# hlesmqh/WS3D

Hardware: AMD Instinct MI355X
Metric: KITTI scenes/sec (16384 pts) Stage-1 RPN fwd, 1/2/4/8 GPU; FPS+group HBM GB/s (higher is better)
Workload: dtype f32

## Files before the change

### include/ws3d_ops.h

```cpp
#ifndef WS3D_OPS_H
#define WS3D_OPS_H

#include <stddef.h>
#include <stdint.h>

#ifdef __cplusplus
extern "C" {
#endif

#define WS3D_OK 0
#define WS3D_E_INVALID (-1)
#define WS3D_E_LAUNCH (-2)
#define WS3D_E_WORKSPACE (-3)
#define WS3D_E_UNSUPPORTED (-4)

#if defined(__GNUC__)
#define WS3D_API __attribute__((visibility("default")))
#else
#define WS3D_API
#endif

typedef void *ws3d_stream_t;

#define WS3D_ABI_VERSION 6
// ... 168 lines not shown
                                        size_t workspace_bytes, ws3d_stream_t stream);
WS3D_API int ws3d_three_interpolate_grad_det(int b, int c, int n, int m, const float *grad_out, const int32_t *idx,
                                             const float *weight, float *grad_points, void *workspace,
                                             size_t workspace_bytes, ws3d_stream_t stream);

WS3D_API int ws3d_bias_act_inplace(int b, int o_ch, long l, int relu, float *y, const float *bias,
                                   ws3d_stream_t stream);

WS3D_API int ws3d_rowmax_bias_act(int b, int o_ch, long m, int s, int relu, const float *y, const float *bias,
                                  float *out, ws3d_stream_t stream);

WS3D_API int ws3d_query_and_group_nlc(int b, int n, int m, int c, float radius, int nsample, int use_xyz,
                                      const float *xyz, const float *new_xyz, const float *features_nlc,
                                      int32_t *idx_out, float *out_nlc, const void *sorted, ws3d_stream_t stream);
WS3D_API int ws3d_three_interpolate_nlc(int b, int c, int m, int n, const float *feats_nlc, const int32_t *idx,
                                        const float *weight, float *out_nlc, int out_stride, ws3d_stream_t stream);
WS3D_API int ws3d_rowmax_rows(long rows_out, int ns, int o_ch, const float *y, float *out, int out_stride,
                              ws3d_stream_t stream);

WS3D_API int ws3d_sa_mlp3_pool(long rows, int nsample, int c1, int c2, int c3, const float *x_rows4,
                               const float *w1t, const float *b1, const float *w2t, const float *b2,
                               const float *w3t, const float *b3, int relu3, float *out, int out_stride,
                               ws3d_stream_t stream);

WS3D_API int ws3d_mlp2_rows(long rows, int k_dim, int o1, int o2, const float *x_rows, const float *w1t, const float *b1, int relu1,
                   const float *w2t, const float *b2, int relu2, float *out, int *ticket, ws3d_stream_t stream);

WS3D_API size_t ws3d_rpn_heads_blob_bytes(int o2);
WS3D_API int ws3d_rpn_heads_pack(int o2, const float *w1t, const float *b1, int relu1, const float *w2t, const float *b2, int relu2, void *blob,
                        ws3d_stream_t stream);
WS3D_API int ws3d_rpn_heads(long rows, const float *x_rows, int heads, const void *blob_cls, float *out_cls, int *ticket_cls, int o2_reg,
                   const void *blob_reg, float *out_reg, int *ticket_reg, int workgroups, ws3d_stream_t stream);

WS3D_API int ws3d_qinterp_gemm(int b, int n, int m, int c, int o_dim, const float *q, const int32_t *idx, const float *weight, const float *lin,
                      const float *skip, int c1, const float *wb, const float *b1, int relu1, const float *w2t, const float *b2, int relu2,
                      float *out, ws3d_stream_t stream);


WS3D_API int ws3d_boxes_overlap_bev(int num_a, const float *boxes_a, int num_b, const float *boxes_b,
                           float *ans, ws3d_stream_t stream);

WS3D_API int ws3d_boxes_iou_bev(int num_a, const float *boxes_a, int num_b, const float *boxes_b,
                       float *ans, ws3d_stream_t stream);

WS3D_API int ws3d_nms_mask(int boxes_num, const float *boxes, float thresh, int normal, int full_grid,
                  uint64_t *mask, ws3d_stream_t stream);

WS3D_API size_t ws3d_nms_workspace_bytes(int boxes_num);
WS3D_API int ws3d_nms(int boxes_num, const float *boxes, float thresh, int normal, int max_keep,
                      void *workspace, size_t workspace_bytes, int64_t *keep, int32_t *num_keep,
                      ws3d_stream_t stream);

WS3D_API int ws3d_nms_batched(int batch, int boxes_num, const float *boxes, float thresh, int normal,
                              int max_keep, void *workspace, size_t workspace_bytes, int64_t *keep,
                              int32_t *num_keep, ws3d_stream_t stream);


WS3D_API int ws3d_radius_nms_batched(int batch, int n, const float *centers, float radius, int max_keep,
                                     void *workspace, size_t workspace_bytes, int64_t *keep,
                                     int32_t *num_keep, ws3d_stream_t stream);

WS3D_API int ws3d_topk_sorted(int b, int n, int k, const float *scores, float *out_scores, int64_t *out_idx,
                              ws3d_stream_t stream);
WS3D_API size_t ws3d_topk_workspace_bytes(int b, int n);
WS3D_API int ws3d_topk_sorted_ws(int b, int n, int k, const float *scores, float *out_scores, int64_t *out_idx, void *workspace,
                                 size_t workspace_bytes, ws3d_stream_t stream);
// ... 78 lines not shown
```

### ws3d_amd/_lib.py

```python
from __future__ import annotations

import ctypes as C
import os

_HERE = os.path.dirname(os.path.abspath(__file__))
DIST_MODE = int(os.environ.get("WS3D_DIST_MODE", "0") or 0)
LIB_PATH = os.environ.get("WS3D_HIP_LIB") or os.path.join(
    _HERE, "libws3d_hip.so" if DIST_MODE == 0 else "libws3d_hip_dm%d.so" % DIST_MODE)

E_INVALID, E_LAUNCH, E_WORKSPACE, E_UNSUPPORTED = -1, -2, -3, -4
ABI_VERSION = 6

_vp = C.c_void_p
_i = C.c_int
_f = C.c_float
_sz = C.c_size_t

class CompactMlpArgs(C.Structure):
    _fields_ = [("b", _i), ("n", _i), ("m", _i), ("max_rows", C.c_long), ("o1", _i), ("o2", _i), ("o3", _i), ("pmat", _vp), ("p_stride", _i),
                ("xyz", _vp), ("new_xyz", _vp), ("rowc", _vp), ("rowsrc", _vp), ("total", _vp), ("w1x", _vp), ("b1", _vp), ("relu1", _i),
                ("w2t", _vp), ("b2", _vp), ("relu2", _i), ("w3t", _vp), ("b3", _vp), ("mid", _vp), ("out", _vp), ("out_stride", _i), ("limit", C.c_long)]


SIGNATURES = {
# ... 14 lines not shown
    "ws3d_ball_query_pairs2": (_i, [_i, _i, _i, _vp, _vp, _vp, C.c_float, _i, _vp, _vp, _vp, _vp, C.c_float, _i, _vp, _vp, _vp, _vp, _vp]),
    "ws3d_sorted_points_bytes": (_sz, [_i, _i]),
    "ws3d_sort_points_x": (_i, [_i, _i, _vp, _vp, _vp]),
    "ws3d_sort_points_xz": (_i, [_i, _i, _vp, _vp, _vp]),
    "ws3d_sort_points_grid": (_i, [_i, _i, _vp, _vp, _vp]),
    "ws3d_sort_points_jobs": (_i, [_i, _i, _vp, _vp, _vp, _vp, _vp]),
    "ws3d_group_points": (_i, [_i, _i, _i, _i, _i, _vp, _vp, _vp, _vp]),
    "ws3d_group_points_grad": (_i, [_i, _i, _i, _i, _i, _vp, _vp, _vp, _vp]),
    "ws3d_query_and_group": (_i, [_i, _i, _i, _i, _f, _i, _i, _vp, _vp, _vp, _vp, _vp, _vp, _vp]),
    "ws3d_three_nn": (_i, [_i, _i, _i, _vp, _vp, _vp, _vp, _vp, _vp]),
    "ws3d_three_interpolate": (_i, [_i, _i, _i, _i, _vp, _vp, _vp, _vp, _vp]),
    "ws3d_three_interpolate_grad": (_i, [_i, _i, _i, _i, _vp, _vp, _vp, _vp, _vp]),
    "ws3d_bn_workspace_bytes": (C.c_size_t, [_i, _i, C.c_long]),
    "ws3d_bn_relu_train_fwd": (_i, [_i, _i, C.c_long, _vp, _vp, _vp, C.c_float, C.c_float, _i, _vp, _vp, _vp, _vp, _vp, _vp,
                                    _vp, C.c_size_t, _vp]),
    "ws3d_bn_relu_train_bwd": (_i, [_i, _i, C.c_long, _vp, _vp, _vp, _vp, _vp, _vp, _i, _vp, _vp, _vp, _vp, C.c_size_t, _vp]),
    "ws3d_conv1x1_wgrad_workspace_bytes": (C.c_size_t, [_i, _i, _i, C.c_long]),
    "ws3d_conv1x1_wgrad": (_i, [_i, _i, _i, C.c_long, _vp, _vp, _vp, _vp, C.c_size_t, _vp]),
    "ws3d_gemm_pool": (_i, [C.c_long, _i, _i, _i, _vp, _vp, _vp, _i, _vp, _i, _vp, C.c_long, _vp]),
    "ws3d_pool_nsample": (_i, [C.c_long, _i, _vp, _vp, _vp, _vp]),
    "ws3d_pool_nsample_grad": (_i, [C.c_long, _i, _vp, _vp, _vp, _vp]),
    "ws3d_scatter_workspace_bytes": (C.c_size_t, [_i, _i, _i, C.c_long]),
    "ws3d_group_points_grad_det": (_i, [_i, _i, _i, _i, _i, _vp, _vp, _vp, _vp, C.c_size_t, _vp]),
    "ws3d_three_interpolate_grad_det": (_i, [_i, _i, _i, _i, _vp, _vp, _vp, _vp, _vp, C.c_size_t, _vp]),
    "ws3d_query_and_group_nlc": (_i, [_i, _i, _i, _i, _f, _i, _i, _vp, _vp, _vp, _vp, _vp, _vp, _vp]),
    "ws3d_three_interpolate_nlc": (_i, [_i, _i, _i, _i, _vp, _vp, _vp, _vp, _i, _vp]),
    "ws3d_rowmax_rows": (_i, [C.c_long, _i, _i, _vp, _vp, _i, _vp]),
    "ws3d_sa_mlp3_pool": (_i, [C.c_long, _i, _i, _i, _i, _vp, _vp, _vp, _vp, _vp, _vp, _vp, _i, _vp, _i, _vp]),
    "ws3d_qinterp_gemm": (_i, [_i, _i, _i, _i, _i, _vp, _vp, _vp, _vp, _vp, _i, _vp, _vp, _i, _vp, _vp, _i, _vp, _vp]),
    "ws3d_mlp2_rows": (_i, [C.c_long, _i, _i, _i, _vp, _vp, _vp, _i, _vp, _vp, _i, _vp, _vp, _vp]),
    "ws3d_rpn_heads_blob_bytes": (_sz, [_i]),
    "ws3d_rpn_heads_pack": (_i, [_i, _vp, _vp, _i, _vp, _vp, _i, _vp, _vp]),
    "ws3d_rpn_heads": (_i, [C.c_long, _vp, _i, _vp, _vp, _vp, _i, _vp, _vp, _vp, _i, _vp]),
    "ws3d_decode_center_boxes": (_i, [_i, _i, _i, _f, _f, _f, _f, _f, _vp, _vp, _vp, _vp]),
    "ws3d_topk_sorted": (_i, [_i, _i, _i, _vp, _vp, _vp, _vp]),
    "ws3d_topk_workspace_bytes": (C.c_size_t, [_i, _i]),
    "ws3d_topk_sorted_ws": (_i, [_i, _i, _i, _vp, _vp, _vp, _vp, C.c_size_t, _vp]),
    "ws3d_topk_sorted_sigmoid": (_i, [_i, _i, _i, _vp, _vp, _vp, _vp]),
    "ws3d_topk_sorted_sigmoid_ws": (_i, [_i, _i, _i, _vp, _vp, _vp, _vp, C.c_size_t, _vp]),
    "ws3d_three_nn_weights": (_i, [C.c_long, _vp, _vp, _vp]),
    "ws3d_three_nn_w": (_i, [_i, _i, _i, _vp, _vp, _vp, _vp, _vp, _vp, _vp]),
    "ws3d_three_nn_wq": (_i, [_i, _i, _i, _vp, _vp, _vp, _vp, _vp, _vp, _vp, _vp]),
    "ws3d_three_nn_jobs": (_i, [_i, _i, _vp, _vp, _vp, _vp, _vp, _vp, _vp, _vp, _vp]),
    "ws3d_bias_act_inplace": (_i, [_i, _i, C.c_long, _i, _vp, _vp, _vp]),
    "ws3d_rowmax_bias_act": (_i, [_i, _i, C.c_long, _i, _i, _vp, _vp, _vp, _vp]),
    "ws3d_boxes_overlap_bev": (_i, [_i, _vp, _i, _vp, _vp, _vp]),
    "ws3d_boxes_iou_bev": (_i, [_i, _vp, _i, _vp, _vp, _vp]),
    "ws3d_nms_mask": (_i, [_i, _vp, _f, _i, _i, _vp, _vp]),
    "ws3d_nms_workspace_bytes": (_sz, [_i]),
    "ws3d_nms": (_i, [_i, _vp, _f, _i, _i, _vp, _sz, _vp, _vp, _vp]),
    "ws3d_nms_batched": (_i, [_i, _i, _vp, _f, _i, _i, _vp, _sz, _vp, _vp, _vp]),
    "ws3d_radius_nms_batched": (_i, [_i, _i, _vp, _f, _i, _vp, _sz, _vp, _vp, _vp]),
    "ws3d_gather_gemm": (_i, [_i, _i, _i, _i, _i, _i, _vp, _vp, _vp, _vp, _vp, _vp, _i, _vp, _vp]),
    "ws3d_gather_gemm2": (_i, [_i, _i, _i, _i, _i, _i, _i, _vp, _vp, _vp, _vp, _vp, _vp, _i, _vp, _vp, _i, _vp, _vp]),
    "ws3d_pgather_gemm2": (_i, [_i, _i, _i, _i, _i, _i, _vp, _i, _vp, _vp, _vp, _vp, _vp, _i, _vp, _vp, _i, _vp, _vp, C.c_long, _vp]),
    "ws3d_pgather_rows": (_i, [_i, _i, _i, _i, _i, _vp, _i, _vp, _vp, _vp, _vp, _vp, _i, _vp, _vp]),
    "ws3d_qinterp_rows": (_i, [_i, _i, _i, _i, _vp, _vp, _vp, _vp, _vp, _i, _vp, _vp, _i, _vp, _vp]),
    "ws3d_compact_pairs": (_i, [C.c_long, _i, _vp, _vp, _vp, _vp, _vp]),
    "ws3d_compact_pairs_count": (_i, [C.c_long, _i, _vp, _vp, _vp]),
    "ws3d_compact_pairs_rows": (_i, [C.c_long, _i, _vp, _vp, _vp, _vp, _vp, _vp, _vp]),
    "ws3d_pgather_gemm2_compact": (_i, [_i, _i, _i, C.c_long, _i, _i, _vp, _i, _vp, _vp, _vp, _vp, _vp, _vp, _vp, _i, _vp, _vp, _i, _vp, C.c_long, _vp]),
    "ws3d_pgather_gemm3_compact": (_i, [_i, _i, _i, C.c_long, _i, _i, _i, _vp, _i, _vp, _vp, _vp, _vp, _vp, _vp, _vp, _i, _vp, _vp, _i, _vp, _vp, _vp, _i, C.c_long, _vp]),
    "ws3d_gemm_pool_compact": (_i, [C.c_long, _i, _i, _vp, _vp, _vp, _vp, _vp, _vp, _i, C.c_long, _vp]),
    "ws3d_compact_mlp_pair": (_i, [_i, C.POINTER(CompactMlpArgs), C.POINTER(CompactMlpArgs), _vp]),
    "ws3d_chain_mlp3_ticket_ints": (_i, []),
    "ws3d_chain_mlp3_blob_floats": (_sz, [_i]),
# ... 65 lines not shown
```

### ws3d_amd/build.py

```python
from __future__ import annotations

import argparse
import concurrent.futures as cf
import glob
import os
import shutil
import subprocess
import sys

HERE = os.path.dirname(os.path.abspath(__file__))
CSRC = os.path.join(HERE, "csrc")
OBJ = os.path.join(CSRC, "build")
LIB = os.path.join(HERE, "libws3d_hip.so")
DIST_MODES = (0, 1, 2)


def lib_path(dist_mode: int = 0) -> str:
    return LIB if dist_mode == 0 else os.path.join(HERE, "libws3d_hip_dm%d.so" % dist_mode)
ARCH = "gfx950"
SOURCES = ["core.hip", "fps.hip", "fps_v3.hip", "fps_bucket.hip", "fps_nested.hip", "ballquery_group.hip", "interpolate.hip", "roipool3d.hip", "iou3d.hip", "proposals.hip", "scatter_det.hip", "sa_mlp.hip", "bn_relu.hip", "gemm_pool.hip", "conv_wgrad.hip", "chain_mlp.hip", "rpn_heads.hip", "kitti_eval.hip", "instance_clouds.hip"]
CXXFLAGS = ["-O3", "-std=c++17", "-fPIC", "-ffp-contract=off", "-fno-fast-math",
            "-fvisibility=hidden", "-Wall", "-Wno-unused-function"]


def hipcc() -> str:
    for cand in (os.environ.get("HIPCC"), shutil.which("hipcc"), "/opt/rocm/bin/hipcc"):
        if cand and os.path.exists(cand):
            return cand
    raise RuntimeError("hipcc not found (looked at $HIPCC, PATH, /opt/rocm/bin)")


def _deps(src: str):
    return [src, *glob.glob(os.path.join(CSRC, "*.h")), os.path.join(HERE, "..", "include", "ws3d_ops.h"),
            os.path.join(CSRC, "exports.map"), os.path.abspath(__file__)]


def _compile(src: str, force: bool, verbose: bool, dist_mode: int = 0) -> str:
    path = os.path.join(CSRC, src)
    obj = os.path.join(OBJ if dist_mode == 0 else OBJ + "_dm%d" % dist_mode, os.path.splitext(src)[0] + ".o")
    if not force and os.path.exists(obj) and all(
            os.path.getmtime(obj) >= os.path.getmtime(d) for d in _deps(path)):
        return obj
    cmd = [hipcc(), f"--offload-arch={ARCH}", *CXXFLAGS, f"-DWS3D_DIST_MODE={dist_mode}", *os.environ.get("WS3D_EXTRA_DEFS", "").split(), "-c", path, "-o", obj]
    if verbose:
        print(" ".join(cmd), flush=True)
    r = subprocess.run(cmd, capture_output=True, text=True)
    if r.returncode != 0:
        raise RuntimeError(f"hipcc failed for {src}:\n{r.stdout}\n{r.stderr}")
    if verbose and r.stderr.strip():
        print(r.stderr)
    return obj


# ... 43 lines not shown
```

### ws3d_amd/compat.py

```python
from __future__ import annotations

import sys
import types

import os

import torch

from . import _lib
from ._lib import Ws3dError, check


def _dev(*tensors):
    dev = None
    for t in tensors:
        if t is None:
            continue
        if not t.is_cuda:
            raise Ws3dError("ws3d_amd ops need HIP ('cuda') tensors; there is no CPU fallback")
        if not t.is_contiguous():
            raise Ws3dError("ws3d_amd ops need contiguous tensors (the reference asserts the same)")
        if dev is None:
            dev = t.device
        elif t.device != dev:
# ... 753 lines not shown
    if n == 0 or tuple(w1t.shape) != (128, 128) or w2t.size(0) != 128 or not w1t.is_contiguous() or not w2t.is_contiguous():
        return None
    for b, nm, o in ((b1, "b1", 128), (b2, "b2", O2)):
        if b is not None:
            _f32(b, nm)
            if b.numel() != o or not b.is_contiguous():
                return None
    blob = torch.empty((n + 15) // 16 * 4, dtype=torch.float32, device=dev)
    with _on(dev):
        check(_lib.load().ws3d_rpn_heads_pack(O2, _p(w1t), _p(b1), int(bool(relu1)), _p(w2t), _p(b2), int(bool(relu2)), _p(blob), _stream()),
              "rpn_heads_pack")
    return blob


def rpn_heads(x2d, heads, blob_cls, blob_reg, o2_reg, tickets, workgroups=0):
    dev = _dev(x2d)
    _f32(x2d, "x2d")
    if (x2d.dim() != 2 or x2d.size(1) != 128 or x2d.size(0) % 32 or not x2d.is_contiguous() or heads not in (1, 2, 3) or
            tickets is None or tickets.dtype != torch.int32 or tickets.numel() < 2 or not tickets.is_contiguous()):
        return None
    R = x2d.size(0)
    out_cls = torch.empty((R, 1), dtype=torch.float32, device=dev) if heads & 1 else None
    out_reg = torch.empty((R, int(o2_reg)), dtype=torch.float32, device=dev) if heads & 2 else None
    with _on(dev):
        rc = _lib.load().ws3d_rpn_heads(R, _p(x2d), int(heads), _p(blob_cls) if heads & 1 else None, _p(out_cls), _p(tickets[0:1]),
                                        int(o2_reg) if heads & 2 else 0, _p(blob_reg) if heads & 2 else None, _p(out_reg), _p(tickets[1:2]),
                                        int(workgroups), _stream())
    if rc == _lib.E_UNSUPPORTED:
        return None
    check(rc, "rpn_heads")
    return out_cls, out_reg


def pool_nsample(x):
    dev = _dev(x)
    _f32(x, "x")
    ns = x.size(-1)
    out = torch.empty(x.shape[:-1], dtype=torch.float32, device=dev)
    arg = torch.empty(x.shape[:-1], dtype=torch.uint8, device=dev)
    with _on(dev):
        check(_lib.load().ws3d_pool_nsample(out.numel(), ns, _p(x), _p(out), _p(arg), _stream()), "pool_nsample")
    return out, arg


def pool_nsample_grad(grad_out, arg, nsample):
    dev = _dev(grad_out, arg)
    _f32(grad_out, "grad_out")
    if arg.dtype != torch.uint8 or not arg.is_contiguous():
        raise TypeError("arg must be a contiguous uint8 tensor")
    grad_x = torch.empty(tuple(grad_out.shape) + (nsample,), dtype=torch.float32, device=dev)
    with _on(dev):
        check(_lib.load().ws3d_pool_nsample_grad(grad_out.numel(), nsample, _p(grad_out), _p(arg), _p(grad_x), _stream()),
              "pool_nsample_grad")
    return grad_x


SA_MLP3_SHAPES = {(16, 16, 32), (32, 32, 64)}


def sa_mlp3_pool(x_rows4, nsample, layers, out, col0=0):
    (w1, b1, r1), (w2, b2, r2), (w3, b3, r3) = layers
    widths = (w1.size(1), w2.size(1), w3.size(1))
    if (x_rows4.size(1) != 4 or widths not in SA_MLP3_SHAPES or nsample not in (16, 32) or not (r1 and r2)
            or b1 is None or b2 is None or b3 is None):
        return False
    dev = _dev(x_rows4, out)
# ... 507 lines not shown
```

### ws3d_amd/fastpath.py

```python
from __future__ import annotations

import contextlib
import contextvars

import torch
import torch.nn as nn

from . import compat as _C
from . import nn_blocks, pn2_ops

FUSED_SA_MLP = True
SA1_FROM_LISTS = True
FUSED_GEMM_POOL = True
FUSED_INTERP_GEMM = True
NESTED_FPS = True
GEOMETRY_AHEAD = True
_AHEAD_OVERRIDE = contextvars.ContextVar("ws3d_geometry_ahead", default=None)


@contextlib.contextmanager
def geometry_ahead(on: bool):
    token = _AHEAD_OVERRIDE.set(bool(on))
    try:
        yield
# ... 9 lines not shown
    finally:
        _COMPACT_ONLY.reset(token)


def primed_compact_scales(net, pointcloud: torch.Tensor, margin: float = None):
    margin = PRIMED_MARGIN if margin is None else margin
    keys, per_level = set(), {}
    for row in list_fill(net, pointcloud):
        si = per_level.get(row["level"], 0)
        per_level[row["level"]] = si + 1
        if row["fill"] <= margin * COMPACT_MAX_FILL:
            keys.add((row["level"] - 1, si))
    return frozenset(keys)


def _geometry_ahead_now() -> bool:
    v = _AHEAD_OVERRIDE.get()
    return GEOMETRY_AHEAD if v is None else v
GEOMETRY_IN_CAPTURE = False
PER_POINT_L1 = True
COMPACT_MAX_FILL = 0.55
COMPACT_PAIRS = True
PAIR_DISPATCH = "device"
PRIMED_MARGIN = 0.85
_COMPACT_ONLY = contextvars.ContextVar("ws3d_compact_only_scales", default=frozenset())
CHAIN_MLP = True
PAIRED_SCALES = True
MERGED_THREE_NN = True
FUSED_PROLOGUE = True
MERGED_BINNING = True
PER_POINT_FP = True
FUSED_MLP2_ROWS = True
FUSED_HEADS = True
FUSED_GATHER_GEMM2 = True
BIN_INPUT_AHEAD = True
FUSED_QINTERP_GEMM_MIN_ROWS = 30000
FUSED_COMPACT3_MAX_LDS = 64 * 1024
FUSED_GATHER_GEMM = True
GRID_MIN_N = 256
DUAL_SCALE_SEARCH = True
NESTED_CHAIN = True
QUERY_CELL_ORDER = True
PARALLEL_SCALES = True
PARALLEL_HEADS = True


def _row_weights(block):
    w, shift, act = block._folded()
    if act is not None and not isinstance(act, nn.ReLU):
        raise NotImplementedError("fast path supports ReLU / no activation only")
    cache = block.__dict__.get("_row_cache")
    if cache is None or cache[0] is not w:
        cache = (w, w.t().contiguous())
        if not torch.cuda.is_current_stream_capturing():
            block.__dict__["_row_cache"] = cache
    return cache[1], shift, act is not None


def _row_weights_xyz_last(block):
    wt, bias, relu = _row_weights(block)
    cache = block.__dict__.get("_row_cache_xyz_last")
    if cache is None or cache[0] is not wt:
        cache = (wt, torch.cat((wt[3:], wt[:3]), dim=0).contiguous())
        if not torch.cuda.is_current_stream_capturing():
            block.__dict__["_row_cache_xyz_last"] = cache
    return cache[1], bias, relu


def _split_rows(block, wt: torch.Tensor, c2: int):
    cache = block.__dict__.get("_split_cache")
    if cache is None or cache[0] is not wt or cache[1] != c2:
        cache = (wt, c2, wt[:c2].contiguous(), wt[c2:].contiguous())
        if not torch.cuda.is_current_stream_capturing():
            block.__dict__["_split_cache"] = cache
    return cache[2], cache[3]


def _layer(x2d: torch.Tensor, block) -> torch.Tensor:
    wt, bias, relu = _row_weights(block)
    if bias is None:
        y = torch.mm(x2d, wt)
        return torch.relu_(y) if relu else y
    if relu:
        return torch._addmm_activation(bias, x2d, wt, use_gelu=False)
    return torch.addmm(bias, x2d, wt)


def _blocks(seq):
    return [m for m in seq if isinstance(m, nn_blocks._ConvBlock)]


def mlp_rows(x2d: torch.Tensor, seq, ticket=None) -> torch.Tensor:
    blocks = _blocks(seq)
    if FUSED_MLP2_ROWS and len(blocks) == 2 and x2d.size(1) == 128 and x2d.is_contiguous():
        (w1, b1, r1), (w2, b2, r2) = _row_weights(blocks[0]), _row_weights(blocks[1])
        y = _C.mlp2_rows(x2d, w1, b1, r1, w2, b2, r2, ticket)
        if y is not None:
            return y
    for blk in blocks:
        x2d = _layer(x2d, blk)
    return x2d


def _heads_blob(seq):
    blocks = _blocks(seq)
    if len(blocks) != 2:
        return None
    (w1, b1, r1), (w2, b2, r2) = _row_weights(blocks[0]), _row_weights(blocks[1])
    cache = blocks[0].__dict__.get("_heads_blob")
    if cache is None or cache[0] is not w1 or cache[1] is not b1 or cache[2] is not w2 or cache[3] is not b2:
        cache = (w1, b1, w2, b2, _C.rpn_heads_pack(w1, b1, r1, w2, b2, r2), w2.size(1))
        if not torch.cuda.is_current_stream_capturing():
# ... 94 lines not shown
def _arena_for(net, B: int, device, extra: int = 0, clear: bool = True) -> _ZeroArena:
    n = extra + 64
    if COMPACT_PAIRS:
        for sa in net.SA_modules:
            n += B * sa.npoint * sum(_blocks(mlp)[-1].conv.out_channels for mlp in sa.mlps) + 4
            n += 4 * len(sa.groupers)
        if CHAIN_MLP:
            n += _C.chain_ticket_ints() + 4
    return _ZeroArena(n, device, clear)


class _PairList:
    __slots__ = ("nbr", "pairs")

    def __init__(self, nbr, pairs):
        self.nbr, self.pairs = nbr, pairs


def _per_point_l1(sa, feats: torch.Tensor, nbrs):
    B, N, C = feats.shape
    wts = [(_row_weights_xyz_last(_blocks(mlp)[0])[0] if nbr is not None else None) for mlp, nbr in zip(sa.mlps, nbrs)]
    cache = sa.__dict__.get("_pp_cache")
    if cache is None or len(cache[0]) != len(wts) or any(a is not b for a, b in zip(cache[0], wts)):
        used = [w for w in wts if w is not None]
        wcat = torch.cat([w[:C] for w in used], dim=1).contiguous()
        offs, w1xs, o = [], [], 0
        for w in wts:
            offs.append(o if w is not None else -1)
            w1xs.append(w[C:C + 3].contiguous() if w is not None else None)
            o += w.size(1) if w is not None else 0
        cache = (wts, wcat, offs, w1xs)
        if not torch.cuda.is_current_stream_capturing():
            sa.__dict__["_pp_cache"] = cache
    return torch.mm(feats.view(B * N, C), cache[1]), cache[2], cache[3]


def _lists_and_pairs(radius, nsample, xyz, new_xyz, sorted_xyz, zeros=None):
    total = zeros.take((1,), torch.int32) if zeros is not None else None
    both = _C.ball_query_pairs(radius, nsample, xyz, new_xyz, sorted_xyz, total)
    if both is not None:
        return both
    nbr = _C.ball_query_lists(radius, nsample, xyz, new_xyz, sorted_xyz)
    return nbr, _C.compact_pairs(nbr)


def _neighbour_lists(sa, xyz, new_xyz, sorted_xyz, c_feat: int, zeros=None):
    B = xyz.size(0)
    lists = []
    want_pairs = [(_gather_gemm_ok(sa, g, _blocks(mlp), c_feat, B) and COMPACT_PAIRS and PER_POINT_L1 and _blocks(mlp)[0].conv.out_channels <= 256
                   and len(_blocks(mlp)) == 3) for g, mlp in zip(sa.groupers, sa.mlps)]
    if DUAL_SCALE_SEARCH and len(want_pairs) == 2 and all(want_pairs) and sorted_xyz is not None:
        totals = [zeros.take((1,), torch.int32) for _ in range(2)] if zeros is not None else None
        both = _C.ball_query_pairs2([g.radius for g in sa.groupers], [g.nsample for g in sa.groupers], xyz, new_xyz, sorted_xyz, totals)
        if both is not None:
            return [_PairList(nbr, pairs) for nbr, pairs in both]
    for grouper, mlp in zip(sa.groupers, sa.mlps):
        if not _gather_gemm_ok(sa, grouper, _blocks(mlp), c_feat, B):
            lists.append(None)
            continue
        if COMPACT_PAIRS and PER_POINT_L1 and _blocks(mlp)[0].conv.out_channels <= 256 and len(_blocks(mlp)) == 3:
            nbr, pairs = _lists_and_pairs(grouper.radius, grouper.nsample, xyz, new_xyz, sorted_xyz, zeros)
            lists.append(_PairList(nbr, pairs))
        else:
            lists.append(_C.ball_query_lists(grouper.radius, grouper.nsample, xyz, new_xyz, sorted_xyz))
    return lists


# ... 235 lines not shown

    if run_paired():
        pass
    elif geo is not None and geo.aux is not None and PARALLEL_SCALES and len(widths) == 2:
        if PER_POINT_L1 and any(n is not None and len(_blocks(m)) >= 3 for n, m in zip(nbrs, sa.mlps)):
            pp[0] = _per_point_l1(sa, feats, nbrs)
        fork = torch.cuda.Event()
        fork.record(geo.main)
        geo.aux.wait_event(fork)
        with torch.cuda.stream(geo.aux):
            run_scale(1)
            join = torch.cuda.Event()
            join.record(geo.aux)
        run_scale(0)
        geo.main.wait_event(join)
    else:
        for si in range(len(widths)):
            run_scale(si)
    return new_xyz, out.view(B, sa.npoint, -1)


def fp_forward(fp, unknown: torch.Tensor, known: torch.Tensor, unknown_feats, known_feats: torch.Tensor, nn3=None, sorted_unknown=None,
               known_xz=None):
    B, n = unknown.size(0), unknown.size(1)
    idx, weight = nn3 if nn3 is not None else _C.three_nn_with_weights(unknown, known, known_xz[0] if known_xz is not None else pn2_ops.sort_points_xz(known),
                                                                        sorted_unknown if QUERY_CELL_ORDER else None)
    c2 = known_feats.size(2)
    c1 = 0 if unknown_feats is None else unknown_feats.size(2)
    blocks = _blocks(fp.mlp)
    if PER_POINT_FP and blocks and blocks[0].conv.out_channels % 4 == 0:
        wt1, b1, r1 = _row_weights(blocks[0])
        wa, wb = _split_rows(blocks[0], wt1, c2)
        m = known_feats.size(1)
        q = torch.mm(known_feats.reshape(B * m, c2), wa).view(B, m, -1)
        fuse2 = len(blocks) == 2 and B * n >= FUSED_QINTERP_GEMM_MIN_ROWS
        if fuse2:
            wt2, b2, r2 = _row_weights(blocks[1])
        if c1 > 4:
            lin = torch.mm(unknown_feats.reshape(B * n, c1), wb) if b1 is None else torch.addmm(b1, unknown_feats.reshape(B * n, c1), wb)
            y = _C.qinterp_gemm(q, idx, weight, wt2, b2, r2, lin=lin, relu=r1) if fuse2 else None
            if y is not None:
                return y.view(B, n, -1)
            y = _C.qinterp_rows(q, idx, weight, lin=lin, relu=r1)
        else:
            sk = None if c1 == 0 else unknown_feats.contiguous()
            y = _C.qinterp_gemm(q, idx, weight, wt2, b2, r2, skip=sk, wb=wb if c1 else None, bias=b1, relu=r1) if fuse2 else None
            if y is not None:
                return y.view(B, n, -1)
            y = _C.qinterp_rows(q, idx, weight, skip=sk, wb=wb if c1 else None, bias=b1, relu=r1)
        if y is not None:
            for blk in blocks[1:]:
                y = _layer(y, blk)
            return y.view(B, n, -1)
    if FUSED_INTERP_GEMM and blocks and blocks[0].conv.out_channels % 64 == 0 and B * n >= 8192:
        wt1, b1, r1 = _row_weights(blocks[0])
        y = _C.interp_gemm(known_feats.contiguous(), None if unknown_feats is None else unknown_feats.contiguous(), idx, weight, wt1, b1, r1)
        if y is not None:
            for blk in blocks[1:]:
                y = _layer(y, blk)
            return y.view(B, n, -1)
    cat = torch.empty((B, n, c2 + c1), dtype=torch.float32, device=unknown.device)
    _C.three_interpolate_nlc(known_feats, idx, weight, cat)
    if c1:
        cat[:, :, c2:] = unknown_feats
    return mlp_rows(cat.view(B * n, c2 + c1), fp.mlp).view(B, n, -1)


@torch.no_grad()
def backbone_forward(net, pointcloud: torch.Tensor, zeros: _ZeroArena = None):
    if FUSED_PROLOGUE and pointcloud.is_cuda and pointcloud.dim() == 3 and pointcloud.is_contiguous() and pointcloud.size(-1) > 3:
        if zeros is None:
            zeros = _arena_for(net, pointcloud.size(0), pointcloud.device, clear=False)
# ... 93 lines not shown
```

### ws3d_amd/pipeline.py

```python
from __future__ import annotations

import os
from typing import Iterable, Iterator, Tuple

import numpy as np
import torch

from . import roipool3d_ops, stage1


def ensure_hw_queues(n: int = 32) -> bool:
    if torch.cuda.is_initialized():
        return False
    os.environ.setdefault("GPU_MAX_HW_QUEUES", str(n))
    return True


def _hw_queue_cap() -> int:
    try:
        return int(os.environ.get("GPU_MAX_HW_QUEUES", "4"))
    except ValueError:
        return 4


# ... 100 lines not shown
    def _prime(self, slot: dict) -> None:
        slot["primed"] = True
        if not self.use_graph or self.graph_error is not None:
            return
        prev = self._tunable(True)
        try:
            with _LaunchGeometry(self.depth >= THROUGHPUT_GEOMETRY_MIN_DEPTH):
                self._prime_capture(slot)
        finally:
            if prev is not None:
                torch.cuda.tunable.enable(prev[0])
                torch.cuda.tunable.tuning_enable(prev[1])

    def _prime_capture(self, slot: dict) -> None:
        try:
            stream = slot["stream"]
            stream.wait_stream(torch.cuda.current_stream(self.device))
            from . import fastpath
            if self.compact_only is None:
                with torch.cuda.stream(stream):
                    blank = not bool(slot["inp"].any().item())
                    self.compact_only = (fastpath.primed_compact_scales(self.model.rpn.backbone_net, slot["inp"])
                                         if (self.pair_dispatch == "primed" and not blank) else frozenset())
                    self.compact_only_source = "blank input: both forms kept" if blank else ("fills of the first primed batch" if self.pair_dispatch == "primed" else "pair_dispatch=device")
            with fastpath.geometry_ahead(False), fastpath.compact_only_scales(self.compact_only), torch.cuda.stream(stream):
                for _ in range(2):
                    self.body(slot["inp"], slot["exchange"])
            stream.synchronize()
            graph = torch.cuda.CUDAGraph()
            with fastpath.compact_only_scales(self.compact_only), torch.cuda.graph(graph, stream=stream):
                slot["out"] = self.body(slot["inp"], slot["exchange"])
            slot["graph"] = graph
            slot["heads_blobs"] = fastpath.heads_blobs(self.model.rpn)
        except Exception as exc:
            self.graph_error = repr(exc)
            slot["graph"] = None

    def capture_all(self) -> bool:
        for slot in self.slots:
            if not slot["primed"]:
                slot["inp"].copy_(self.slots[0]["inp"])
                self._prime(slot)
        torch.cuda.synchronize(self.device)
        return self.use_graph and self.graph_error is None

    @torch.no_grad()
    def submit(self, pts=None) -> int:
        slot = self.slots[self.submitted % self.depth]
        with torch.cuda.device(self.device):
            if pts is not None:
                t = torch.from_numpy(np.ascontiguousarray(pts, dtype=np.float32)) if not torch.is_tensor(pts) else pts
                if t.size(0) > self.B or tuple(t.shape[1:]) != tuple(slot["inp"].shape[1:]):
                    raise ValueError(f"batch of shape {tuple(t.shape)} does not fit the pipeline's {tuple(slot['inp'].shape)}")
            if not slot["primed"]:
                if pts is not None:
                    slot["inp"][:t.size(0)].copy_(t)
                    if t.size(0) < self.B:
                        slot["inp"][t.size(0):] = slot["inp"][t.size(0) - 1]
                self._prime(slot)
            if pts is not None and t.is_cuda:
                slot["stream"].wait_stream(torch.cuda.current_stream(self.device))
                t.record_stream(slot["stream"])
            with torch.cuda.stream(slot["stream"]):
                if pts is not None:
                    slot["inp"][:t.size(0)].copy_(t, non_blocking=True)
                    if t.size(0) < self.B:
# ... 33 lines not shown
```

Baseline: 6816.

## Add split-bf16 MFMA row GEMM with prepacked weights for FP/SA layers

Adds a custom HIP GEMM that splits each fp32 operand into three bf16 parts and runs six bf16 MFMA products per k-block, which emulates fp32 precision on the matrix cores. Weights are prepacked once per module and cached. Activations are converted on the fly into double-buffered LDS. The kernel replaces torch.mm/addmm in the per-layer row MLP, the SA pointwise projection and the interpolation weight GEMMs, with a shape fallback to the library path. The trade is six times the MFMA work and some loss of exactness against fp32 SGEMM, in exchange for matrix-core throughput instead of vector FMAs.

```diff
diff --git a/include/ws3d_ops.h b/include/ws3d_ops.h
--- a/include/ws3d_ops.h
+++ b/include/ws3d_ops.h
@@ -224,6 +224,11 @@
 WS3D_API int ws3d_rpn_heads(long rows, const float *x_rows, int heads, const void *blob_cls, float *out_cls, int *ticket_cls, int o2_reg,
                    const void *blob_reg, float *out_reg, int *ticket_reg, int workgroups, ws3d_stream_t stream);
 
+WS3D_API size_t ws3d_gemm_rows_pack_bytes(int k_dim, int n_dim);
+WS3D_API int ws3d_gemm_rows_pack(int k_dim, int n_dim, const float *wt, void *pack, ws3d_stream_t stream);
+WS3D_API int ws3d_gemm_rows_split(long rows, int k_dim, int n_dim, const float *a, const void *pack, const float *bias, int relu, float *out,
+                         ws3d_stream_t stream);
+
 WS3D_API int ws3d_qinterp_gemm(int b, int n, int m, int c, int o_dim, const float *q, const int32_t *idx, const float *weight, const float *lin,
                       const float *skip, int c1, const float *wb, const float *b1, int relu1, const float *w2t, const float *b2, int relu2,
                       float *out, ws3d_stream_t stream);
diff --git a/ws3d_amd/_lib.py b/ws3d_amd/_lib.py
--- a/ws3d_amd/_lib.py
+++ b/ws3d_amd/_lib.py
@@ -70,6 +70,9 @@
     "ws3d_rpn_heads_blob_bytes": (_sz, [_i]),
     "ws3d_rpn_heads_pack": (_i, [_i, _vp, _vp, _i, _vp, _vp, _i, _vp, _vp]),
     "ws3d_rpn_heads": (_i, [C.c_long, _vp, _i, _vp, _vp, _vp, _i, _vp, _vp, _vp, _i, _vp]),
+    "ws3d_gemm_rows_pack_bytes": (_sz, [_i, _i]),
+    "ws3d_gemm_rows_pack": (_i, [_i, _i, _vp, _vp, _vp]),
+    "ws3d_gemm_rows_split": (_i, [C.c_long, _i, _i, _vp, _vp, _vp, _i, _vp, _vp]),
     "ws3d_decode_center_boxes": (_i, [_i, _i, _i, _f, _f, _f, _f, _f, _vp, _vp, _vp, _vp]),
     "ws3d_topk_sorted": (_i, [_i, _i, _i, _vp, _vp, _vp, _vp]),
     "ws3d_topk_workspace_bytes": (C.c_size_t, [_i, _i]),
diff --git a/ws3d_amd/build.py b/ws3d_amd/build.py
--- a/ws3d_amd/build.py
+++ b/ws3d_amd/build.py
@@ -18,7 +18,7 @@
 def lib_path(dist_mode: int = 0) -> str:
     return LIB if dist_mode == 0 else os.path.join(HERE, "libws3d_hip_dm%d.so" % dist_mode)
 ARCH = "gfx950"
-SOURCES = ["core.hip", "fps.hip", "fps_v3.hip", "fps_bucket.hip", "fps_nested.hip", "ballquery_group.hip", "interpolate.hip", "roipool3d.hip", "iou3d.hip", "proposals.hip", "scatter_det.hip", "sa_mlp.hip", "bn_relu.hip", "gemm_pool.hip", "conv_wgrad.hip", "chain_mlp.hip", "rpn_heads.hip", "kitti_eval.hip", "instance_clouds.hip"]
+SOURCES = ["core.hip", "fps.hip", "fps_v3.hip", "fps_bucket.hip", "fps_nested.hip", "ballquery_group.hip", "interpolate.hip", "roipool3d.hip", "iou3d.hip", "proposals.hip", "scatter_det.hip", "sa_mlp.hip", "bn_relu.hip", "gemm_pool.hip", "conv_wgrad.hip", "chain_mlp.hip", "rpn_heads.hip", "gemm_rows.hip", "kitti_eval.hip", "instance_clouds.hip"]
 CXXFLAGS = ["-O3", "-std=c++17", "-fPIC", "-ffp-contract=off", "-fno-fast-math",
             "-fvisibility=hidden", "-Wall", "-Wno-unused-function"]
 
diff --git a/ws3d_amd/compat.py b/ws3d_amd/compat.py
--- a/ws3d_amd/compat.py
+++ b/ws3d_amd/compat.py
@@ -809,6 +809,44 @@
     return out_cls, out_reg
 
 
+def gemm_rows_pack(wt):
+    dev = _dev(wt)
+    _f32(wt, "wt")
+    if wt.dim() != 2:
+        return None
+    K, N = wt.shape
+    n = int(_lib.load().ws3d_gemm_rows_pack_bytes(K, N))
+    if n == 0:
+        return None
+    pack = torch.empty((n + 15) // 16 * 4, dtype=torch.float32, device=dev)
+    with _on(dev):
+        check(_lib.load().ws3d_gemm_rows_pack(K, N, _p(wt), _p(pack), _stream()), "gemm_rows_pack")
+    return pack
+
+
+def gemm_rows_split(x2d, pack, n_dim, bias=None, relu=False, out=None):
+    if pack is None or x2d.dim() != 2 or not x2d.is_contiguous() or (bias is not None and (not bias.is_contiguous() or bias.numel() != n_dim)):
+        return None
+    dev = _dev(x2d, pack, bias, out)
+    _f32(x2d, "x2d")
+    R, K = x2d.shape
+    n_dim = int(n_dim)
+    if R % 64 or K % 32 or n_dim % 64 or pack.numel() * pack.element_size() < K * n_dim * 6:
+        return None
+    if bias is not None:
+        _f32(bias, "bias")
+    if out is None:
+        out = torch.empty((R, n_dim), dtype=torch.float32, device=dev)
+    elif tuple(out.shape) != (R, n_dim) or out.dtype != torch.float32:
+        return None
+    with _on(dev):
+        rc = _lib.load().ws3d_gemm_rows_split(R, K, n_dim, _p(x2d), _p(pack), _p(bias), int(bool(relu)), _p(out), _stream())
+    if rc == _lib.E_UNSUPPORTED:
+        return None
+    check(rc, "gemm_rows_split")
+    return out
+
+
 def pool_nsample(x):
     dev = _dev(x)
     _f32(x, "x")
diff --git a/ws3d_amd/csrc/gemm_rows.hip b/ws3d_amd/csrc/gemm_rows.hip
--- /dev/null
+++ b/ws3d_amd/csrc/gemm_rows.hip
@@ -0,0 +1,224 @@
+#include "common.h"
+
+namespace ws3d {
+
+typedef float rows_f16 __attribute__((ext_vector_type(16)));
+typedef __bf16 rows_bf8 __attribute__((ext_vector_type(8)));
+typedef unsigned rows_u4 __attribute__((ext_vector_type(4)));
+typedef float rows_f4 __attribute__((ext_vector_type(4)));
+
+constexpr int GR_THREADS = 256;
+constexpr int GR_TM = 64;
+constexpr int GR_KB = 32;
+constexpr int GR_FRAG = 1024;
+#ifndef WS3D_GR_TALL_MIN_TILES
+#define WS3D_GR_TALL_MIN_TILES 512
+#endif
+constexpr int GR_TALL_MIN_TILES = WS3D_GR_TALL_MIN_TILES;
+constexpr int GR_MAX_DIM = 4096;
+__host__ __device__ constexpr int gr_tile_rows(int nbt, int mbw) { return nbt == 4 ? 32 * mbw : 64 * mbw; }
+__host__ __device__ constexpr int gr_a_stage(int tm) { return tm / 32 * 2 * 3 * GR_FRAG; }
+__host__ __device__ constexpr int gr_lds_bytes(int tm) { return 2 * gr_a_stage(tm); }
+static_assert(gr_lds_bytes(128) <= 64 * 1024 && gr_lds_bytes(128) * 2 <= 160 * 1024, "inside the default per-workgroup cap, two workgroups per CU");
+
+__device__ __forceinline__ void rows_split3(float x, __bf16 &p1, __bf16 &p2, __bf16 &p3) {
+    p1 = (__bf16)x;
+    const float r1 = x - (float)p1;
+    p2 = (__bf16)r1;
+    const float r2 = r1 - (float)p2;
+    p3 = (__bf16)r2;
+}
+
+__device__ __forceinline__ void rows_split8(const float *v, rows_bf8 &q1, rows_bf8 &q2, rows_bf8 &q3) {
+#pragma unroll
+    for (int j = 0; j < 8; ++j) {
+        __bf16 p1, p2, p3;
+        rows_split3(v[j], p1, p2, p3);
+        q1[j] = p1; q2[j] = p2; q3[j] = p3;
+    }
+}
+
+__device__ __forceinline__ float rows_relu(float y) { return y < 0.f ? 0.f : y; }
+
+__global__ __launch_bounds__(256) void gemm_rows_pack_kernel(int K, int N, const float *__restrict__ wt, rows_u4 *__restrict__ pack) {
+    const int nb_all = N / 32;
+    const long total = (long)(K / GR_KB) * nb_all * 2 * 64;
+    for (long i = (long)blockIdx.x * blockDim.x + threadIdx.x; i < total; i += (long)gridDim.x * blockDim.x) {
+        const int lane = (int)(i & 63), s = (int)((i >> 6) & 1);
+        const long f = i >> 7;
+        const int nb = (int)(f % nb_all), kb = (int)(f / nb_all);
+        const int col = nb * 32 + (lane & 31), k0 = kb * GR_KB + 16 * s + 8 * (lane >> 5);
+        float v[8];
+#pragma unroll
+        for (int j = 0; j < 8; ++j) v[j] = wt[(long)(k0 + j) * N + col];
+        rows_bf8 q1, q2, q3;
+        rows_split8(v, q1, q2, q3);
+        rows_u4 *dst = pack + ((f * 2 + s) * 3) * 64 + lane;
+        dst[0] = __builtin_bit_cast(rows_u4, q1);
+        dst[64] = __builtin_bit_cast(rows_u4, q2);
+        dst[128] = __builtin_bit_cast(rows_u4, q3);
+    }
+}
+
+template <int NBT, int MBW>
+__global__ __launch_bounds__(GR_THREADS, 2) void gemm_rows_kernel(int K, int N, int ntn, const float *__restrict__ a, const rows_u4 *__restrict__ pack,
+                                                                  const float *__restrict__ bias, int relu, float *__restrict__ out) {
+    extern __shared__ __attribute__((aligned(16))) unsigned char smem_rows[];
+    constexpr int TM = gr_tile_rows(NBT, MBW);
+    constexpr int UNITS = TM / 64;
+    constexpr int STAGE = gr_a_stage(TM);
+    const int tid = threadIdx.x, w = tid >> 6, lane = tid & 63, r = lane & 31, h = lane >> 5;
+    const int tn = (int)(blockIdx.x % (unsigned)ntn);
+    const long tm = blockIdx.x / (unsigned)ntn;
+    const int nb_all = N / 32, nkb = K / GR_KB;
+    const int nbl = NBT == 4 ? w : (w & 1), mb0 = NBT == 4 ? 0 : (w >> 1) * MBW;
+
+    const int srow = (lane & 7) + 8 * (lane >> 5) + 16 * w, skq = (lane >> 3) & 3;
+    const rows_f4 *ap = reinterpret_cast<const rows_f4 *>(a + (tm * TM + srow) * (long)K + 8 * skq);
+    const size_t a_unit = (size_t)16 * K;
+    const int a_wr = ((srow >> 5) * 2 + (skq >> 1)) * 3 * GR_FRAG + ((skq & 1) * 32 + (srow & 31)) * 16;
+    const rows_u4 *wp = pack + (size_t)(tn * NBT + nbl) * 6 * 64 + lane;
+    const size_t w_kb = (size_t)nb_all * 6 * 64;
+
+    rows_f16 acc[MBW];
+#pragma unroll
+    for (int m = 0; m < MBW; ++m)
+#pragma unroll
+        for (int i = 0; i < 16; ++i) acc[m][i] = 0.f;
+    rows_u4 wc[6];
+#pragma unroll
+    for (int i = 0; i < 6; ++i) wc[i] = rows_u4{0u, 0u, 0u, 0u};
+
+    for (int kb = -1; kb < nkb; ++kb) {
+        const bool more = kb + 1 < nkb;
+        rows_f4 ra[UNITS][2];
+        rows_u4 wn[6];
+        if (more) {
+#pragma unroll
+            for (int u = 0; u < UNITS; ++u) {
+                ra[u][0] = ap[u * a_unit + (kb + 1) * (GR_KB / 4)];
+                ra[u][1] = ap[u * a_unit + (kb + 1) * (GR_KB / 4) + 1];
+            }
+#pragma unroll
+            for (int i = 0; i < 6; ++i) wn[i] = wp[(kb + 1) * w_kb + i * 64];
+        }
+        if (kb >= 0) {
+            const unsigned char *buf = smem_rows + (kb & 1) * STAGE + lane * 16;
+#pragma unroll
+            for (int s = 0; s < 2; ++s) {
+                const rows_bf8 w1 = __builtin_bit_cast(rows_bf8, wc[3 * s]), w2 = __builtin_bit_cast(rows_bf8, wc[3 * s + 1]),
+                               w3 = __builtin_bit_cast(rows_bf8, wc[3 * s + 2]);
+                rows_bf8 a1[MBW], a2[MBW], a3[MBW];
+#pragma unroll
+                for (int m = 0; m < MBW; ++m) {
+                    const unsigned char *af = buf + ((mb0 + m) * 2 + s) * 3 * GR_FRAG;
+                    a1[m] = *reinterpret_cast<const rows_bf8 *>(af);
+                    a2[m] = *reinterpret_cast<const rows_bf8 *>(af + GR_FRAG);
+                    a3[m] = *reinterpret_cast<const rows_bf8 *>(af + 2 * GR_FRAG);
+                }
+#pragma unroll
+                for (int m = 0; m < MBW; ++m) acc[m] = __builtin_amdgcn_mfma_f32_32x32x16_bf16(w3, a1[m], acc[m], 0, 0, 0);
+#pragma unroll
+                for (int m = 0; m < MBW; ++m) acc[m] = __builtin_amdgcn_mfma_f32_32x32x16_bf16(w2, a2[m], acc[m], 0, 0, 0);
+#pragma unroll
+                for (int m = 0; m < MBW; ++m) acc[m] = __builtin_amdgcn_mfma_f32_32x32x16_bf16(w1, a3[m], acc[m], 0, 0, 0);
+#pragma unroll
+                for (int m = 0; m < MBW; ++m) acc[m] = __builtin_amdgcn_mfma_f32_32x32x16_bf16(w2, a1[m], acc[m], 0, 0, 0);
+#pragma unroll
+                for (int m = 0; m < MBW; ++m) acc[m] = __builtin_amdgcn_mfma_f32_32x32x16_bf16(w1, a2[m], acc[m], 0, 0, 0);
+#pragma unroll
+                for (int m = 0; m < MBW; ++m) acc[m] = __builtin_amdgcn_mfma_f32_32x32x16_bf16(w1, a1[m], acc[m], 0, 0, 0);
+            }
+        }
+        if (more) {
+            unsigned char *nxt = smem_rows + ((kb + 1) & 1) * STAGE + a_wr;
+#pragma unroll
+            for (int u = 0; u < UNITS; ++u) {
+                const float v[8] = {ra[u][0][0], ra[u][0][1], ra[u][0][2], ra[u][0][3], ra[u][1][0], ra[u][1][1], ra[u][1][2], ra[u][1][3]};
+                rows_bf8 q1, q2, q3;
+                rows_split8(v, q1, q2, q3);
+                *reinterpret_cast<rows_bf8 *>(nxt + u * 12 * GR_FRAG) = q1;
+                *reinterpret_cast<rows_bf8 *>(nxt + u * 12 * GR_FRAG + GR_FRAG) = q2;
+                *reinterpret_cast<rows_bf8 *>(nxt + u * 12 * GR_FRAG + 2 * GR_FRAG) = q3;
+            }
+#pragma unroll
+            for (int i = 0; i < 6; ++i) wc[i] = wn[i];
+        }
+        __syncthreads();
+    }
+
+    const int n0 = (tn * NBT + nbl) * 32 + 4 * h;
+    rows_f4 b4[4];
+    if (bias) {
+#pragma unroll
+        for (int g = 0; g < 4; ++g) b4[g] = *reinterpret_cast<const rows_f4 *>(bias + n0 + 8 * g);
+    }
+#pragma unroll
+    for (int m = 0; m < MBW; ++m) {
+        float *orow = out + (tm * TM + (mb0 + m) * 32 + r) * (long)N + n0;
+#pragma unroll
+        for (int g = 0; g < 4; ++g) {
+            rows_f4 y;
+#pragma unroll
+            for (int e = 0; e < 4; ++e) y[e] = acc[m][4 * g + e];
+            if (bias) y = y + b4[g];
+            if (relu) {
+#pragma unroll
+                for (int e = 0; e < 4; ++e) y[e] = rows_relu(y[e]);
+            }
+            *reinterpret_cast<rows_f4 *>(orow + 8 * g) = y;
+        }
+    }
+}
+
+static bool gr_dims_ok(int K, int N) { return K >= GR_KB && K <= GR_MAX_DIM && K % GR_KB == 0 && N >= 64 && N <= GR_MAX_DIM && N % 64 == 0; }
+
+}
+
+extern "C" size_t ws3d_gemm_rows_pack_bytes(int k_dim, int n_dim) {
+    return ws3d::gr_dims_ok(k_dim, n_dim) ? (size_t)k_dim * n_dim * 6 : 0;
+}
+
+extern "C" int ws3d_gemm_rows_pack(int k_dim, int n_dim, const float *wt, void *pack, ws3d_stream_t stream) {
+    using namespace ws3d;
+    if (!wt || !pack || (reinterpret_cast<uintptr_t>(pack) & 15) || (reinterpret_cast<uintptr_t>(wt) & 3)) {
+        set_error("ws3d_gemm_rows_pack: invalid argument");
+        return WS3D_E_INVALID;
+    }
+    if (!gr_dims_ok(k_dim, n_dim)) {
+        set_error("ws3d_gemm_rows_pack: unsupported shape K=%d N=%d (K %% 32, N %% 64, both <= %d)", k_dim, n_dim, GR_MAX_DIM);
+        return WS3D_E_UNSUPPORTED;
+    }
+    const long threads = (long)(k_dim / GR_KB) * (n_dim / 32) * 128;
+    hipLaunchKernelGGL(gemm_rows_pack_kernel, dim3((unsigned)((threads + 255) / 256)), dim3(256), 0, as_stream(stream), k_dim, n_dim, wt,
+                       static_cast<rows_u4 *>(pack));
+    return check_launch("ws3d_gemm_rows_pack");
+}
+
+extern "C" int ws3d_gemm_rows_split(long rows, int k_dim, int n_dim, const float *a, const void *pack, const float *bias, int relu, float *out,
+                                    ws3d_stream_t stream) {
+    using namespace ws3d;
+    if (rows < 0 || k_dim <= 0 || n_dim <= 0 || !a || !pack || !out) {
+        set_error("ws3d_gemm_rows_split: invalid argument (rows=%ld K=%d N=%d)", rows, k_dim, n_dim);
+        return WS3D_E_INVALID;
+    }
+    const uintptr_t al = reinterpret_cast<uintptr_t>(a) | reinterpret_cast<uintptr_t>(pack) | reinterpret_cast<uintptr_t>(out) | reinterpret_cast<uintptr_t>(bias);
+    const int nbt = n_dim % 128 == 0 ? 4 : 2;
+    if (!gr_dims_ok(k_dim, n_dim) || rows % GR_TM || (al & 15) || (rows / GR_TM) * (n_dim / (32 * nbt)) > 0x7fffffffL) {
+        set_error("ws3d_gemm_rows_split: unsupported shape or alignment (rows=%ld K=%d N=%d; rows %% 64, K %% 32, N %% 64, 16-byte pointers)", rows,
+                  k_dim, n_dim);
+        return WS3D_E_UNSUPPORTED;
+    }
+    if (rows == 0) return WS3D_OK;
+    const int ntn = n_dim / (32 * nbt);
+    const bool tall = nbt == 4 && rows % 128 == 0 && (rows / 128) * ntn >= GR_TALL_MIN_TILES;
+    const int tm = tall ? 128 : 64;
+    const unsigned grid = (unsigned)((rows / tm) * ntn);
+    auto go = [&](auto kern) -> int {
+        hipLaunchKernelGGL(kern, dim3(grid), dim3(GR_THREADS), (size_t)gr_lds_bytes(tm), as_stream(stream), k_dim, n_dim, ntn, a,
+                           static_cast<const rows_u4 *>(pack), bias, relu ? 1 : 0, out);
+        return WS3D_OK;
+    };
+    if (int rc = nbt == 2 ? go(gemm_rows_kernel<2, 1>) : tall ? go(gemm_rows_kernel<4, 4>) : go(gemm_rows_kernel<4, 2>)) return rc;
+    return check_launch("ws3d_gemm_rows_split");
+}
diff --git a/ws3d_amd/fastpath.py b/ws3d_amd/fastpath.py
--- a/ws3d_amd/fastpath.py
+++ b/ws3d_amd/fastpath.py
@@ -65,6 +65,7 @@
 PER_POINT_FP = True
 FUSED_MLP2_ROWS = True
 FUSED_HEADS = True
+SPLIT_GEMMS = True
 FUSED_GATHER_GEMM2 = True
 BIN_INPUT_AHEAD = True
 FUSED_QINTERP_GEMM_MIN_ROWS = 30000
@@ -109,8 +110,37 @@
     return cache[2], cache[3]
 
 
+_SPLIT_GEMM_LIBRARY_WINS = frozenset({(512, 1024, 512)})
+
+
+def _split_gemm_wins(rows: int, k: int, n: int) -> bool:
+    return (rows, k, n) not in _SPLIT_GEMM_LIBRARY_WINS
+
+
+def _split_gemm(x2d: torch.Tensor, holder, key: str, wt: torch.Tensor, bias=None, relu: bool = False):
+    if not SPLIT_GEMMS or x2d.dim() != 2 or not _split_gemm_wins(x2d.size(0), wt.size(0), wt.size(1)):
+        return None
+    packs = holder.__dict__.get("_gemm_rows_packs")
+    ent = None if packs is None else packs.get(key)
+    if ent is None or ent[0] is not wt:
+        if torch.cuda.is_current_stream_capturing():
+            return None
+        ent = (wt, _C.gemm_rows_pack(wt))
+        holder.__dict__.setdefault("_gemm_rows_packs", {})[key] = ent
+    if ent[1] is None:
+        return None
+    return _C.gemm_rows_split(x2d, ent[1], wt.size(1), bias, relu)
+
+
+def gemm_rows_packs(model):
+    return [ent[1] for m in model.modules() for ent in m.__dict__.get("_gemm_rows_packs", {}).values() if ent[1] is not None]
+
+
 def _layer(x2d: torch.Tensor, block) -> torch.Tensor:
     wt, bias, relu = _row_weights(block)
+    y = _split_gemm(x2d, block, "row", wt, bias, relu)
+    if y is not None:
+        return y
     if bias is None:
         y = torch.mm(x2d, wt)
         return torch.relu_(y) if relu else y
@@ -271,7 +301,8 @@
         cache = (wts, wcat, offs, w1xs)
         if not torch.cuda.is_current_stream_capturing():
             sa.__dict__["_pp_cache"] = cache
-    return torch.mm(feats.view(B * N, C), cache[1]), cache[2], cache[3]
+    p = _split_gemm(feats.view(B * N, C), sa, "pp", cache[1])
+    return (p if p is not None else torch.mm(feats.view(B * N, C), cache[1])), cache[2], cache[3]
 
 
 def _lists_and_pairs(radius, nsample, xyz, new_xyz, sorted_xyz, zeros=None):
@@ -573,12 +604,15 @@
         wt1, b1, r1 = _row_weights(blocks[0])
         wa, wb = _split_rows(blocks[0], wt1, c2)
         m = known_feats.size(1)
-        q = torch.mm(known_feats.reshape(B * m, c2), wa).view(B, m, -1)
+        q = _split_gemm(known_feats.reshape(B * m, c2), blocks[0], "wa", wa)
+        q = (q if q is not None else torch.mm(known_feats.reshape(B * m, c2), wa)).view(B, m, -1)
         fuse2 = len(blocks) == 2 and B * n >= FUSED_QINTERP_GEMM_MIN_ROWS
         if fuse2:
             wt2, b2, r2 = _row_weights(blocks[1])
         if c1 > 4:
-            lin = torch.mm(unknown_feats.reshape(B * n, c1), wb) if b1 is None else torch.addmm(b1, unknown_feats.reshape(B * n, c1), wb)
+            lin = _split_gemm(unknown_feats.reshape(B * n, c1), blocks[0], "wb", wb, b1)
+            if lin is None:
+                lin = torch.mm(unknown_feats.reshape(B * n, c1), wb) if b1 is None else torch.addmm(b1, unknown_feats.reshape(B * n, c1), wb)
             y = _C.qinterp_gemm(q, idx, weight, wt2, b2, r2, lin=lin, relu=r1) if fuse2 else None
             if y is not None:
                 return y.view(B, n, -1)
diff --git a/ws3d_amd/pipeline.py b/ws3d_amd/pipeline.py
--- a/ws3d_amd/pipeline.py
+++ b/ws3d_amd/pipeline.py
@@ -156,6 +156,7 @@
                 slot["out"] = self.body(slot["inp"], slot["exchange"])
             slot["graph"] = graph
             slot["heads_blobs"] = fastpath.heads_blobs(self.model.rpn)
+            slot["gemm_rows_packs"] = fastpath.gemm_rows_packs(self.model.rpn)
         except Exception as exc:
             self.graph_error = repr(exc)
             slot["graph"] = None
```

Result: faster. 7043, median of 6 (+3.3%).
